# hukenovs/blackman_harris_win

Measured on AMD Instinct MI355X. Metric: window Gsamples/s (BH-7, N=2^26, 32-bit) + fraction of HBM-write roofline, higher is better.
Workload: dtype int64

## Files before the change

blackman_harris_win_amd/csrc/bhw_build.hip:

```cpp
#include "bhw_device.h"

namespace {

template <typename T>
__global__ __launch_bounds__(kBlock) void k_table_build(BhwCordicCfg cfg, uint32_t entries, void *__restrict__ table)
{
    __shared__ T lut_s[32];
    stage_lut<T>(cfg, lut_s);
    const uint32_t u = blockIdx.x * kBlock + threadIdx.x;
    if (u >= entries) return;
    T x, y;
    cordic_q1<T>(lut_s, (T)cfg.x0, (T)((T)u << cfg.z_shl), (int)cfg.n_iter, x, y);
    const int32_t c = (int32_t)(x >> cfg.out_shr), sn = (int32_t)(y >> cfg.out_shr);
    const int2 head = make_int2(__builtin_amdgcn_readfirstlane(c), __builtin_amdgcn_readfirstlane(sn));
    const int4 rec = cfg.tab_dlog > kPackLog ? reinterpret_cast<const int4 *>(cfg.tab_coarse)[u >> fmt_cell_log(cfg.tab_dlog)] : make_int4(0, 0, 0, 0);
    tab_store(table, u, cfg.phi_width - 2 - cfg.z_shr, cfg.tab_split, cfg.tab_dlog, const_cast<void *>(cfg.tab_coarse), c, sn, head, rec,
              cfg.tab_check);
}


template <int NITER, int FMT>
__global__ __launch_bounds__(kBuildThreads) void k_table_build_shared(BhwBuildPlan plan, void *__restrict__ table)
{
    __shared__ int64_t gx[kGroupsPerWg];
    __shared__ int64_t gy[kGroupsPerWg];
    __shared__ int32_t gz[kGroupsPerWg];
    __shared__ int32_t gk[kGroupsPerWg];
    __shared__ uint32_t lut_s[32];
    if (threadIdx.x < 32) lut_s[threadIdx.x] = plan.lut[threadIdx.x];
    __syncthreads();

    constexpr int n_iter = NITER;
    const uint32_t s = plan.z_shl;
    const uint32_t gpw = plan.groups_per_wg;
    const uint32_t group0 = blockIdx.x * gpw;
    const uint32_t n_groups = plan.entries >> 6;

    if (threadIdx.x < gpw) {
        const uint32_t g = group0 + threadIdx.x;
        const uint32_t u_first = g << 6;
        int64_t x = plan.x0, y = plan.x0;
        int32_t zf = (int32_t)((u_first << s) - lut_s[0]);
        const uint32_t span = 63u << s;
        int k = 1;
        bool live = g < n_groups;
        constexpr int kmax = n_iter < kPrefixMax ? n_iter : kPrefixMax;
#pragma unroll
        for (int kk = 1; kk < kmax; ++kk) {
            if (live) {
                const int32_t zl = (int32_t)((uint32_t)zf + span);
                if ((zf < 0) != (zl < 0)) {
                    live = false;
                } else {
                    rot_step(x, y, zf, kk, plan.lut[kk]);
                    k = kk + 1;
                }
            }
        }
        gx[threadIdx.x] = x;
        gy[threadIdx.x] = y;
        gz[threadIdx.x] = zf;
        gk[threadIdx.x] = k;
    }
    __syncthreads();

    const uint32_t wave = __builtin_amdgcn_readfirstlane(threadIdx.x >> 6), lane = threadIdx.x & 63u;
    uint32_t idx_a = lane, idx_m = 64u;
    if (plan.tab_split) {
        const uint32_t e = 1u << plan.log2_entries;
        if (lane & 1u)      { idx_a = (e >> 1) + (lane >> 1); idx_m = 32u; }
        else if (lane & 2u) { idx_a = (e >> 2) + (lane >> 2); idx_m = 16u; }
        else                { idx_a = lane >> 2;              idx_m = 16u; }
    }
    for (uint32_t gi = wave; gi < gpw; gi += kBuildThreads / 64) {
        const uint32_t g = __builtin_amdgcn_readfirstlane(group0 + gi);
        if (g >= n_groups) break;
        int64_t x = gx[gi], y = gy[gi];
        int32_t z = (int32_t)((uint32_t)gz[gi] + (lane << s));
        const int k0 = __builtin_amdgcn_readfirstlane(gk[gi]);
#pragma unroll
        for (int k = 1; k < NITER; ++k) {
            if (k >= kPrefixMax || k >= k0) rot_step(x, y, z, k, plan.lut[k]);
        }
        const int32_t c = (int32_t)(x >> plan.out_shr), sn = (int32_t)(y >> plan.out_shr);
        const int2 head = make_int2(__builtin_amdgcn_readfirstlane(c), __builtin_amdgcn_readfirstlane(sn));
        const uint32_t idx = idx_a + g * idx_m;
        if constexpr (FMT == 4) {
            const uint32_t u = (g << 6) + lane, nmask = 4u * plan.entries - 1u;
            int32_t *d_sin = reinterpret_cast<int32_t *>(table), *d_cos = reinterpret_cast<int32_t *>(const_cast<void *>(plan.tab_coarse));
#pragma unroll
            for (uint32_t q = 0; q < 4u; ++q) {
                int32_t oc, os;
                quadrant_map(q, c, sn, plan.pad0, oc, os);
                const uint32_t i = (q * plan.entries + u - plan.pad) & nmask;
                if (d_sin) d_sin[i] = os;
                if (d_cos) d_cos[i] = oc;
            }
        } else if constexpr (FMT == 0) {
            reinterpret_cast<int2 *>(table)[idx] = make_int2(c, sn);
        } else {
            static_assert(FMT == 1, "k_table_build_shared builds plain and delta16 tables (and the sin / cos sweep) only");
            const int32_t dc = c - head.x, ds = sn - head.y;
            if (plan.check_flag && !(fits_bits(dc, 16) && fits_bits(ds, 16))) atomicOr(plan.check_flag, 1u);
            reinterpret_cast<uint32_t *>(table)[idx] = ((uint32_t)dc & 0xFFFFu) | ((uint32_t)ds << 16);
            if (lane == 0u) reinterpret_cast<int2 *>(const_cast<void *>(plan.tab_coarse))[g] = head;
        }
    }
}

constexpr int kMirrorTail = 6;
constexpr int mirror_gpw(int threads) { return threads / 4; }
constexpr int mirror_heads_max(int threads) { return mirror_gpw(threads) / 2 + 8; }
constexpr int mirror_heads_pad(int threads) { return (mirror_heads_max(threads) + 63) / 64 * 64; }
constexpr int kTailZ = 256;

constexpr int kTailRows = 65;
struct TailD { int8_t v[kTailRows * 64 + 16]; };
constexpr TailD make_tail_d()
{
    TailD t{};
    for (int p = 0; p < 64; ++p)
        for (int v = 0; v < kTailRows; ++v) {
            int d = 0;
            for (int j = 0; j < kMirrorTail; ++j) d += ((p >> j) & 1) ? -(v >> j) : (v >> j);
            t.v[v * 64 + p] = (int8_t)d;
        }
    return t;
}
__device__ const TailD kTailD = make_tail_d();

template <int K, bool ZERO>
__device__ __forceinline__ void rot_narrow(uint32_t &x, uint32_t &y, int32_t &z, uint32_t &zacc, uint32_t lutk)
{
    uint32_t a, b;
    if constexpr (ZERO) {
        asm volatile("v_lshrrev_b32 %[a], %[k], %[y]\n\t"
                     "v_lshrrev_b32 %[b], %[k], %[x]\n\t"
                     "v_min_u32 %[za], %[za], %[z]\n\t"
                     "v_cmpx_gt_i32 vcc, 0, %[z]\n\t"
                     "v_add_u32 %[x], %[x], %[a]\n\t"
                     "v_sub_u32 %[y], %[y], %[b]\n\t"
                     "v_add_u32 %[z], %[z], %[l]\n\t"
                     "s_not_b64 exec, exec\n\t"
                     "v_sub_u32 %[x], %[x], %[a]\n\t"
                     "v_add_u32 %[y], %[y], %[b]\n\t"
                     "v_sub_u32 %[z], %[z], %[l]\n\t"
                     "s_mov_b64 exec, -1"
                     : [x] "+v"(x), [y] "+v"(y), [z] "+v"(z), [za] "+v"(zacc), [a] "=&v"(a), [b] "=&v"(b)
                     : [l] "s"(lutk), [k] "n"(K)
                     : "vcc", "scc");
    } else {
        asm volatile("v_lshrrev_b32 %[a], %[k], %[y]\n\t"
                     "v_lshrrev_b32 %[b], %[k], %[x]\n\t"
                     "v_cmpx_gt_i32 vcc, 0, %[z]\n\t"
                     "v_add_u32 %[x], %[x], %[a]\n\t"
                     "v_sub_u32 %[y], %[y], %[b]\n\t"
                     "v_add_u32 %[z], %[z], %[l]\n\t"
                     "s_not_b64 exec, exec\n\t"
                     "v_sub_u32 %[x], %[x], %[a]\n\t"
                     "v_add_u32 %[y], %[y], %[b]\n\t"
                     "v_sub_u32 %[z], %[z], %[l]\n\t"
                     "s_mov_b64 exec, -1"
                     : [x] "+v"(x), [y] "+v"(y), [z] "+v"(z), [a] "=&v"(a), [b] "=&v"(b)
                     : [l] "s"(lutk), [k] "n"(K)
                     : "vcc", "scc");
    }
}

template <int KA, int NITER>
__device__ __forceinline__ void rot_narrow_block(uint32_t &x, uint32_t &y, int32_t &z, uint32_t &zacc, const uint32_t (&l)[10], int e, uint32_t hi)
{
    uint32_t a, b;
#define BHW_ROT_I(lbl, i, HI_ADD)                                                                                       \
    #lbl ":\n\t"                                                                                                        \
    "v_lshrrev_b32 %[a], %[k" #i "], %[y]\n\t"                                                                          \
    "v_lshrrev_b32 %[b], %[k" #i "], %[x]\n\t"                                                                          \
    HI_ADD                                                                                                             \
    "v_min_u32 %[za], %[za], %[z]\n\t"                                                                                  \
    "v_cmpx_gt_i32 vcc, 0, %[z]\n\t"                                                                                    \
    "v_add_u32 %[x], %[x], %[a]\n\t"                                                                                    \
    "v_sub_u32 %[y], %[y], %[b]\n\t"                                                                                    \
    "v_add_u32 %[z], %[z], %[l" #i "]\n\t"                                                                              \
    "s_not_b64 exec, exec\n\t"                                                                                          \
    "v_sub_u32 %[x], %[x], %[a]\n\t"                                                                                    \
    "v_add_u32 %[y], %[y], %[b]\n\t"                                                                                    \
    "v_sub_u32 %[z], %[z], %[l" #i "]\n\t"                                                                              \
    "s_mov_b64 exec, -1\n"
#define BHW_ROT_PLAIN(i) BHW_ROT_I(i, i, "")
#define BHW_ROT_HI(i) BHW_ROT_I(2##i, i, "v_add_u32 %[b], %[c" #i "], %[b]\n\t")
#define BHW_ROT_DISPATCH(P)                                                                                            \
                 "s_cmp_lt_i32 %[e], 1\n\ts_cbranch_scc1 " #P "0f\n\t"                                                 \
                 "s_cmp_eq_u32 %[e], 1\n\ts_cbranch_scc1 " #P "1f\n\t"                                                 \
                 "s_cmp_eq_u32 %[e], 2\n\ts_cbranch_scc1 " #P "2f\n\t"                                                 \
                 "s_cmp_eq_u32 %[e], 3\n\ts_cbranch_scc1 " #P "3f\n\t"                                                 \
                 "s_cmp_eq_u32 %[e], 4\n\ts_cbranch_scc1 " #P "4f\n\t"                                                 \
                 "s_cmp_eq_u32 %[e], 5\n\ts_cbranch_scc1 " #P "5f\n\t"                                                 \
                 "s_cmp_eq_u32 %[e], 6\n\ts_cbranch_scc1 " #P "6f\n\t"                                                 \
                 "s_cmp_eq_u32 %[e], 7\n\ts_cbranch_scc1 " #P "7f\n\t"                                                 \
                 "s_cmp_eq_u32 %[e], 8\n\ts_cbranch_scc1 " #P "8f\n\t"                                                 \
                 "s_cmp_eq_u32 %[e], 9\n\ts_cbranch_scc1 " #P "9f\n\t"
    constexpr int S = NITER - 1 - KA;
    static_assert(S >= 9 && S <= 30, "bias shifts");
    asm volatile("s_cmp_lg_u32 %[hi], 0\n\ts_cbranch_scc1 100f\n\t"
                 BHW_ROT_DISPATCH()
                 "s_branch 10f\n"
                 BHW_ROT_PLAIN(0) BHW_ROT_PLAIN(1) BHW_ROT_PLAIN(2) BHW_ROT_PLAIN(3) BHW_ROT_PLAIN(4) BHW_ROT_PLAIN(5) BHW_ROT_PLAIN(6) BHW_ROT_PLAIN(7)
                 BHW_ROT_PLAIN(8) BHW_ROT_PLAIN(9)
                 "10:\n\ts_branch 200f\n"
                 "100:\n\t"
                 BHW_ROT_DISPATCH(2)
                 "s_branch 200f\n"
                 BHW_ROT_HI(0) BHW_ROT_HI(1) BHW_ROT_HI(2) BHW_ROT_HI(3) BHW_ROT_HI(4) BHW_ROT_HI(5) BHW_ROT_HI(6) BHW_ROT_HI(7) BHW_ROT_HI(8) BHW_ROT_HI(9)
                 "200:"
                 : [x] "+v"(x), [y] "+v"(y), [z] "+v"(z), [za] "+v"(zacc), [a] "=&v"(a), [b] "=&v"(b)
                 : [e] "s"(e), [hi] "s"(hi), [l0] "s"(l[0]), [l1] "s"(l[1]), [l2] "s"(l[2]), [l3] "s"(l[3]), [l4] "s"(l[4]),
                   [l5] "s"(l[5]), [l6] "s"(l[6]), [l7] "s"(l[7]), [l8] "s"(l[8]), [l9] "s"(l[9]),
                   [k0] "n"(KA), [k1] "n"(KA + 1), [k2] "n"(KA + 2), [k3] "n"(KA + 3), [k4] "n"(KA + 4), [k5] "n"(KA + 5), [k6] "n"(KA + 6),
                   [k7] "n"(KA + 7), [k8] "n"(KA + 8), [k9] "n"(KA + 9),
                   [c0] "n"(1 << S), [c1] "n"(1 << (S - 1)), [c2] "n"(1 << (S - 2)), [c3] "n"(1 << (S - 3)), [c4] "n"(1 << (S - 4)),
                   [c5] "n"(1 << (S - 5)), [c6] "n"(1 << (S - 6)), [c7] "n"(1 << (S - 7)), [c8] "n"(1 << (S - 8)), [c9] "n"(1 << (S - 9))
                 : "vcc", "scc");
#undef BHW_ROT_I
#undef BHW_ROT_PLAIN
#undef BHW_ROT_HI
#undef BHW_ROT_DISPATCH
}

#ifdef BHW_BUILD_STAMPS
__device__ unsigned long long *g_build_stamps = nullptr;
#define BHW_STAMP(i) do { if (g_build_stamps && (threadIdx.x & 63u) == 0u) atomicMax(&g_build_stamps[blockIdx.x * 16u + (i)], (unsigned long long)wall_clock64()); } while (0)
#define BHW_STAMP_MIN(i) do { if (g_build_stamps && threadIdx.x == 0u) g_build_stamps[blockIdx.x * 16u + (i)] = (unsigned long long)wall_clock64(); } while (0)
#else
#define BHW_STAMP(i) do { } while (0)
#define BHW_STAMP_MIN(i) do { } while (0)
#endif

template <int BYTES>
__device__ __forceinline__ void table_store(void *__restrict__ table, uint32_t idx, uint32_t v)
{
    if constexpr (BYTES == 1) asm volatile("global_store_byte %0, %1, %2 sc1" :: "v"(idx), "v"(v), "s"(table) : "memory");
    else asm volatile("global_store_short %0, %1, %2 sc1" :: "v"(idx << 1), "v"(v), "s"(table) : "memory");
}

template <int NITER, int FMT, int THREADS>
__global__ __launch_bounds__(THREADS) __attribute__((amdgpu_waves_per_eu(8, 8))) void k_table_build_mirror(BhwBuildPlan plan, void *__restrict__ table)
{
    BHW_STAMP_MIN(0);
#ifdef BHW_BUILD_STAMPS
    if (g_build_stamps && threadIdx.x == 0u) {
        uint32_t hw, xcc;
        asm volatile("s_getreg_b32 %0, hwreg(HW_REG_HW_ID)\n\ts_getreg_b32 %1, hwreg(HW_REG_XCC_ID)" : "=s"(hw), "=s"(xcc));
        g_build_stamps[blockIdx.x * 16u + 6u] = hw;
        g_build_stamps[blockIdx.x * 16u + 7u] = xcc;
    }
#endif
    static_assert(FMT == 2 || FMT == 3 || FMT == 5, "residual / nibble entries");
    static_assert(NITER >= 21 && NITER <= 32, "narrow state: 32-bit words");
    static_assert(THREADS == 256 || THREADS == 1024, "workgroup shapes");
    constexpr uint32_t gpw = mirror_gpw(THREADS);
    constexpr uint32_t kHeads = mirror_heads_max(THREADS), kHeadsPad = mirror_heads_pad(THREADS);
    static_assert(gpw + 2 * kHeadsPad + 64 <= THREADS, "prefix lanes, two ranges of head chains, the tail-table wave");
    __shared__ int4 gst[gpw];
    __shared__ int2 ghi[gpw];
    __shared__ uint32_t lut_s[32];
    __shared__ uint8_t tail_p[2 * kTailZ];
    __shared__ __attribute__((aligned(16))) int8_t tail_d[kTailRows * 64 + 16];
    constexpr uint32_t kWorkMax = 8 * gpw;
    __shared__ uint32_t work_n;
    __shared__ uint32_t work_u[kWorkMax];
    __shared__ uint32_t esc_n;
    __shared__ int4 esc_list[FMT == 5 ? kEscFill : 1];
    __shared__ int4 esc_tab[FMT == 5 ? kEscSlots : 1];
    if (threadIdx.x < 32) lut_s[threadIdx.x] = plan.lut[threadIdx.x];
    if constexpr (FMT == 5) {
        if (threadIdx.x >= 64u && threadIdx.x < 64u + kEscSlots) esc_tab[threadIdx.x - 64u] = make_int4(-1, 0, 0, 0);
    }
#ifdef BHW_BUILD_STAMPS
    if (g_build_stamps && threadIdx.x == 0u) { asm volatile("s_waitcnt lgkmcnt(0)" ::: "memory"); g_build_stamps[blockIdx.x * 16u + 8u] = (unsigned long long)wall_clock64() | (plan.entries & 0u); }
#endif
    constexpr int n_iter = NITER;
    constexpr int KS = NITER - kMirrorTail;
    const uint32_t s = plan.z_shl;
    const uint32_t group0 = blockIdx.x * gpw;
    const uint32_t E = plan.entries;
    const uint32_t n_groups = E >> 7;
    const uint32_t u_lo = group0 << 6;
    const uint32_t u_hi = ((group0 + gpw) << 6) < (n_groups << 6) ? ((group0 + gpw) << 6) : (n_groups << 6);
    const uint32_t m_last = (E >> 1) - 1u;
    if (threadIdx.x == 0) {
        work_n = 0u;
        esc_n = 0u;
        if (u_hi == (E >> 1)) {
            work_u[0] = E >> 1;
            work_n = 1u;
        }
    }
    if (threadIdx.x >= (uint32_t)THREADS - 64u) {
        const uint32_t t3 = threadIdx.x - ((uint32_t)THREADS - 64u);
#pragma unroll
        for (int q = 0; q < 5; ++q)
            if (t3 + 64u * q < (uint32_t)(kTailRows * 64 + 16) / 16u) reinterpret_cast<int4 *>(tail_d)[t3 + 64u * q] = reinterpret_cast<const int4 *>(kTailD.v)[t3 + 64u * q];
#pragma unroll
        for (int q = 0; q < 2 * kTailZ / 64; ++q) {
            const uint32_t zi = t3 + 64u * (uint32_t)q;
            int32_t z = (int32_t)zi - kTailZ;
            uint32_t p = 0u;
#pragma unroll
            for (int j = 0; j < kMirrorTail; ++j) {
                if (z < 0) { p |= 1u << j; z += (int32_t)plan.lut[KS + j]; } else z -= (int32_t)plan.lut[KS + j];
            }
            tail_p[zi] = (uint8_t)p;
        }
        BHW_STAMP(9);
    }


    __shared__ int32_t hc[2][kHeads], hs[2][kHeads];
    const uint32_t d = fmt_cell_log(plan.tab_dlog);
    const uint32_t cells_total = E >> d;
    uint32_t cell_lo[2] = {0u, 0u}, n_cell[2] = {0u, 0u}, r_lo[2] = {u_lo, 0u}, r_hi[2] = {u_hi, 0u};
    {
        const uint32_t a = u_lo > 1u ? u_lo : 1u, b = (u_hi - 1u) < m_last ? (u_hi - 1u) : m_last;
        if (a <= b) { r_lo[1] = E - b; r_hi[1] = E - a + 1u; }
        if (a <= b && b == (E >> 1) - 1u) r_lo[1] = E >> 1;
    }
#pragma unroll
    for (int w = 0; w < 2; ++w)
        if (r_hi[w] > r_lo[w]) {
            cell_lo[w] = r_lo[w] >> d;
            n_cell[w] = ((r_hi[w] - 1u) >> d) - cell_lo[w] + 1u;
        }
    if (threadIdx.x >= gpw && threadIdx.x < gpw + 2u * kHeadsPad) {
        const uint32_t w = (threadIdx.x - gpw) / kHeadsPad;
        const uint32_t t = (threadIdx.x - gpw) % kHeadsPad;
        if (n_cell[w] && t < n_cell[w] + 2u) {
            const int64_t cell = (t <= n_cell[w]) ? (int64_t)cell_lo[w] + t : (int64_t)cell_lo[w] - 1;
            if (cell >= 0 && cell < (int64_t)cells_total) {
                int64_t x = plan.x0, y = plan.x0;
                int32_t z = (int32_t)((((uint32_t)cell << d) << s) - plan.lut[0]);
#pragma unroll
                for (int r = 1; r < n_iter; ++r) rot_step(x, y, z, r, plan.lut[r]);
                hc[w][t] = (int32_t)(x >> plan.out_shr);
                hs[w][t] = (int32_t)(y >> plan.out_shr);
            }
        }
        BHW_STAMP(10);
    }

    constexpr int kcap = KS < kPrefixMax ? KS : kPrefixMax;
    if (threadIdx.x < gpw) {
        const uint32_t g = group0 + threadIdx.x;
        const uint32_t u_first = g << 6;
        int64_t x = plan.x0, y = plan.x0;
        int32_t zf = (int32_t)((u_first << s) - plan.lut[0]);
        const uint32_t span = 63u << s;
        int k = 1;
        bool live = g < n_groups;
        uint32_t zero0 = 0u;
#pragma unroll
        for (int kk = 1; kk < kcap; ++kk) {
            if (live) {
                const int32_t zl = (int32_t)((uint32_t)zf + span);
                if ((zf < 0) != (zl < 0)) {
                    live = false;
                } else {
                    zero0 |= (uint32_t)(zf == 0);
                    rot_step(x, y, zf, kk, plan.lut[kk]);
                    k = kk + 1;
                }
            }
        }
        const int64_t drift = ((int64_t)1 << (NITER - k + 1)) + 2, lim = (int64_t)1 << NITER;
        const bool narrow = x >= drift && y >= drift && x + drift < lim && y + drift < lim;
        constexpr int64_t kBias = (int64_t)1 << (NITER - 1);
        const bool hi = !narrow && k >= KS - 10 && y >= drift && y + drift < lim && x - kBias >= drift && x - kBias + drift < ((int64_t)1 << 32) &&
                        x + drift < lim + ((int64_t)1 << KS);
        const int64_t xp = hi ? x - kBias : x;
        const uint32_t flags = zero0 | (narrow || hi ? 2u : 0u) | (hi ? 4u : 0u) | (g == 0u ? 8u : 0u);
        gst[threadIdx.x] = make_int4((int32_t)xp, (int32_t)y, zf, (int32_t)((uint32_t)k | (flags << 8)));
        ghi[threadIdx.x] = make_int2((int32_t)(xp >> 32), (int32_t)(y >> 32));
        BHW_STAMP(11);
    }
    BHW_STAMP(1);
    __syncthreads();

    __shared__ int4 hrec[2][kHeads];
    {
        const uint32_t w = threadIdx.x / kHeadsPad, t = threadIdx.x % kHeadsPad;
        if (w < 2u && t < n_cell[w]) {
            const uint32_t cell = cell_lo[w] + t;
            int4 r;
            if (cell + 1u < cells_total) r = make_int4(hc[w][t], hs[w][t], hc[w][t + 1] - hc[w][t], hs[w][t + 1] - hs[w][t]);
            else {
                const uint32_t tp = t ? t - 1u : n_cell[w] + 1u;
                r = make_int4(hc[w][t], hs[w][t], hc[w][t] - hc[w][tp], hs[w][t] - hs[w][tp]);
            }
            if constexpr (FMT == 5) { r.x += (int32_t)kEscBias; r.y += (int32_t)kEscBias; }
            if constexpr (fmt_is_nibble(FMT)) { r.x -= 8; r.y -= 8; }
            hrec[w][t] = r;
            if constexpr (fmt_is_nibble(FMT)) { r.z *= 2; r.w *= 2; }
            if ((cell << d) >= r_lo[w])
                reinterpret_cast<int4 *>(const_cast<void *>(plan.tab_coarse))[cell] = r;
        }
    }
    __syncthreads();
    BHW_STAMP_MIN(2);
    auto record_of = [&](int w, uint32_t cell) -> int4 { return hrec[w][cell - cell_lo[w]]; };

    auto store_entry = [&](auto CHECKED, uint32_t idx, int32_t c, int32_t sn, const int4 rec, uint32_t pos) {
        if constexpr (FMT == 5) {
            const int2 p = tab_predict(rec, pos, d);
            const uint32_t nc = (uint32_t)(c - p.x), ns = (uint32_t)(sn - p.y);
            uint32_t v = nc | (ns << 4);
            if (__builtin_expect((int)(nc - 1u > 14u) | (int)(ns > 15u), 0)) {
                const uint32_t slot = atomicAdd(&esc_n, 1u);
                if (slot < kEscFill) esc_list[slot] = make_int4((int32_t)idx, c, sn, 0);
                v = kEscMarker;
            }
            table_store<1>(table, idx, v);
        } else if constexpr (FMT == 3) {
            const int2 p = tab_predict(rec, pos, d);
            const uint32_t nc = (uint32_t)(c - p.x), ns = (uint32_t)(sn - p.y);
            if constexpr (decltype(CHECKED)::value) {
                if (plan.check_flag && (nc | ns) > 15u) atomicOr(plan.check_flag, 1u);
            }
            table_store<1>(table, idx, nc | (ns << 4));
        } else {
            const int2 p = tab_predict(rec, pos, d);
            const int32_t dc = c - p.x, ds = sn - p.y;
            if constexpr (decltype(CHECKED)::value) {
                if (plan.check_flag && !(fits_bits(dc, 8) && fits_bits(ds, 8))) atomicOr(plan.check_flag, 1u);
            }
            table_store<2>(table, idx, ((uint32_t)dc & 0xFFu) | ((uint32_t)ds << 8));
        }
    };

    const uint32_t wave = __builtin_amdgcn_readfirstlane(threadIdx.x >> 6), lane = threadIdx.x & 63u;
    uint32_t idx_a, idx_m, idx_i;
    if (lane & 1u)      { idx_a = (E >> 1) + (lane >> 1); idx_m = 32u; idx_i = E + (E >> 1) - 1u; }
    else if (lane & 2u) { idx_a = (E >> 2) + (lane >> 2); idx_m = 16u; idx_i = (E >> 1) + (E >> 2) - 1u; }
    else                { idx_a = lane >> 2;              idx_m = 16u; idx_i = E >> 2; }
    if (!plan.tab_split) { idx_a = lane; idx_m = 64u; idx_i = E; }
    const uint32_t fmask = (1u << d) - 1u;
    constexpr uint32_t kWaves = THREADS / 64;
    static_assert(gpw == 16u * kWaves, "a wave walks 16 groups: four at each priority");
    constexpr bool kWholeCells = THREADS % (1 << 9) == 0;
    const uint32_t gi_end = group0 >= n_groups ? 0u : n_groups - group0 < gpw ? n_groups - group0 : gpw;
    const uint32_t zlane = lane << s;
    const uint32_t cell_step = ((uint32_t)THREADS >> d) << 4;
    constexpr int KA = KS - 10;
    static_assert(KA >= 5 && KA < kcap && KS - KA == 10, "ten-rotation block");
    uint32_t rom[10];
#pragma unroll
    for (int i = 0; i < 10; ++i) {
        rom[i] = __builtin_amdgcn_readfirstlane(lut_s[KA + i]);
        asm volatile("" : "+s"(rom[i]));
    }
    auto build_groups = [&](auto CHECKED) {
        uint32_t u = ((group0 + wave) << 6) + lane;
        uint32_t st_off = wave * (uint32_t)sizeof(int4);
        asm volatile("" : "+v"(st_off));
        uint32_t idx = idx_a + (group0 + wave) * idx_m;
        uint32_t off1, pos1, off2, pos2;
        auto cells_of = [&]() {
            const uint32_t um = E - u;
            pos1 = u & fmask;
            off1 = ((u >> d) - cell_lo[0]) << 4;
            pos2 = um & fmask;
            off2 = ((um >> d) - cell_lo[1]) << 4;
        };
        cells_of();
        uint32_t gi = wave;
#pragma unroll 1
        for (uint32_t quarter = 0; quarter < 4u; ++quarter) {
            if (quarter == 0u) __builtin_amdgcn_s_setprio(3);
            else if (quarter == 1u) __builtin_amdgcn_s_setprio(2);
            else if (quarter == 2u) __builtin_amdgcn_s_setprio(1);
            else __builtin_amdgcn_s_setprio(0);
            const uint32_t q_end = (quarter + 1u) * 4u * kWaves < gi_end ? (quarter + 1u) * 4u * kWaves : gi_end;
#pragma unroll 1
            for (; gi < q_end; gi += kWaves) {
                const int4 st = *reinterpret_cast<const int4 *>(reinterpret_cast<const char *>(gst) + st_off);
                const uint32_t kf = __builtin_amdgcn_readfirstlane((uint32_t)st.w);
                const int k0 = (int)(kf & 0xFFu);
                const uint32_t gf = kf >> 8;
                int32_t z = (int32_t)((uint32_t)st.z + zlane);
                uint64_t zmask = 0ull;
                int32_t c1, s1, c2, s2;
                if (gf & 2u) {
                    uint32_t x = (uint32_t)st.x, y = (uint32_t)st.y;
                    uint32_t zacc = ~0u;
                    if (k0 < KA) {
#define BHW_NARROW(K) if constexpr (K < KA) { if (K >= k0) rot_narrow<K, true>(x, y, z, zacc, K < 9 ? (uint32_t)__builtin_amdgcn_readfirstlane(lut_s[K]) : plan.lut[K]); }
                        BHW_NARROW(1) BHW_NARROW(2) BHW_NARROW(3) BHW_NARROW(4) BHW_NARROW(5) BHW_NARROW(6) BHW_NARROW(7) BHW_NARROW(8)
                        BHW_NARROW(9) BHW_NARROW(10) BHW_NARROW(11) BHW_NARROW(12) BHW_NARROW(13) BHW_NARROW(14) BHW_NARROW(15)
#undef BHW_NARROW
                    }
                    const uint32_t hi = (gf >> 2) & 1u;
                    rot_narrow_block<KA, NITER>(x, y, z, zacc, rom, k0 - KA, hi);
                    zmask = __builtin_amdgcn_ballot_w64(zacc == 0u);
                    const uint32_t xrow6 = hi << (NITER - 1 - KS + 6);
                    const uint32_t bias_out = (hi << (NITER - 1)) >> plan.out_shr;
                    static_assert(KS <= 26, "unrolled to rotation 25");
                    constexpr uint32_t lowm = (1u << KS) - 1u;
                    const uint32_t zi = (uint32_t)(z + kTailZ);
                    const uint32_t mx = (x + 128u) & lowm, my = (y + 128u) & lowm;
                    const uint32_t unsafe = (uint32_t)((mx < my ? mx : my) < 256u) | (uint32_t)((zi - 1u) >= (uint32_t)(2 * kTailZ - 1));
                    if (__builtin_expect(__builtin_amdgcn_ballot_w64(unsafe != 0u) == 0ull, 1)) {
                        const uint32_t xx = ((x >> KS) << 6) + xrow6, yy = (y >> KS) << 6;
                        const uint32_t p1 = tail_p[zi], p2 = tail_p[2u * kTailZ - zi];
                        const int32_t dx1 = tail_d[p1 + yy], dy1 = tail_d[p1 + xx], dx2 = tail_d[p2 + xx], dy2 = tail_d[p2 + yy];
                        c1 = (int32_t)(((x - (uint32_t)dx1) >> plan.out_shr) + bias_out);
                        s1 = (int32_t)((y + (uint32_t)dy1) >> plan.out_shr);
                        c2 = (int32_t)((y - (uint32_t)dx2) >> plan.out_shr);
                        s2 = (int32_t)(((x + (uint32_t)dy2) >> plan.out_shr) + bias_out);
                    } else if (hi) {
                        int64_t xw = (int64_t)x + ((int64_t)1 << (NITER - 1)), yw = (int64_t)y;
                        int64_t x2 = yw, y2 = xw;
                        int32_t z2 = -z;
#pragma unroll 1
                        for (int k = KS; k < NITER; ++k) {
                            rot_step_dyn(xw, yw, z, k, lut_s[k], true);
                            rot_step_dyn(x2, y2, z2, k, lut_s[k], true);
                        }
                        c1 = (int32_t)(xw >> plan.out_shr); s1 = (int32_t)(yw >> plan.out_shr);
                        c2 = (int32_t)(x2 >> plan.out_shr); s2 = (int32_t)(y2 >> plan.out_shr);
                    } else {
                        uint32_t x2 = y, y2 = x;
                        int32_t z2 = -z;
                        uint32_t unused = 0u;
#define BHW_NARROW(K) if constexpr (K >= KS && K < NITER) { rot_narrow<K, false>(x, y, z, unused, plan.lut[K]); rot_narrow<K, false>(x2, y2, z2, unused, plan.lut[K]); }
                        BHW_NARROW(15) BHW_NARROW(16) BHW_NARROW(17) BHW_NARROW(18) BHW_NARROW(19) BHW_NARROW(20) BHW_NARROW(21) BHW_NARROW(22)
                        BHW_NARROW(23) BHW_NARROW(24) BHW_NARROW(25) BHW_NARROW(26) BHW_NARROW(27) BHW_NARROW(28) BHW_NARROW(29) BHW_NARROW(30)
                        BHW_NARROW(31)
#undef BHW_NARROW
                        c1 = (int32_t)(x >> plan.out_shr); s1 = (int32_t)(y >> plan.out_shr);
                        c2 = (int32_t)(x2 >> plan.out_shr); s2 = (int32_t)(y2 >> plan.out_shr);
                    }
                } else {
                    const int2 high = ghi[gi];
                    int64_t x = (int64_t)(((uint64_t)(uint32_t)high.x << 32) | (uint32_t)st.x), y = (int64_t)(((uint64_t)(uint32_t)high.y << 32) | (uint32_t)st.y);
#pragma unroll 1
                    for (int k = k0; k < KS; ++k) {
                        zmask |= __builtin_amdgcn_ballot_w64(z == 0);
                        rot_step_dyn(x, y, z, k, lut_s[k], k >= kMad24From);
                    }
                    int64_t x2 = y, y2 = x;
                    int32_t z2 = -z;
#pragma unroll 1
                    for (int k = KS; k < NITER; ++k) {
                        rot_step_dyn(x, y, z, k, lut_s[k], true);
                        rot_step_dyn(x2, y2, z2, k, lut_s[k], true);
                    }
                    c1 = (int32_t)(x >> plan.out_shr); s1 = (int32_t)(y >> plan.out_shr);
                    c2 = (int32_t)(x2 >> plan.out_shr); s2 = (int32_t)(y2 >> plan.out_shr);
                }
                const uint32_t own_idx = fmt_is_nibble(FMT) ? u : idx;
                store_entry(CHECKED, own_idx, c1, s1, *reinterpret_cast<const int4 *>(reinterpret_cast<const char *>(hrec[0]) + off1), pos1);
                auto store_image = [&]() {
                    store_entry(CHECKED, fmt_is_nibble(FMT) ? E - u : idx_i - idx, c2, s2,
                                *reinterpret_cast<const int4 *>(reinterpret_cast<const char *>(hrec[1]) + off2), pos2);
                };
                const uint32_t events = (uint32_t)zmask | (uint32_t)(zmask >> 32) | (gf & 9u);
                if (events == 0u) {
                    store_image();
                } else {
                    const bool replay = u != 0u && ((((zmask >> lane) & 1ull) != 0ull) || ((gf & 1u) && lane == 0u));
                    bool deferred = false;
                    if (replay) {
                        const uint32_t slot = atomicAdd(&work_n, 1u);
                        if (slot < kWorkMax) { work_u[slot] = u; deferred = true; }
                        else {
                            int64_t xf = plan.x0, yf = plan.x0;
                            int32_t zf = (int32_t)(((E - u) << s) - lut_s[0]);
#pragma unroll 1
                            for (int r = 1; r < n_iter; ++r) rot_step_dyn(xf, yf, zf, r, lut_s[r], r >= kMad24From);
                            c2 = (int32_t)(xf >> plan.out_shr);
                            s2 = (int32_t)(yf >> plan.out_shr);
                        }
                    }
                    if (u != 0u && !deferred) store_image();
                }
                u += (uint32_t)THREADS;
                st_off += kWaves * (uint32_t)sizeof(int4);
                idx += kWaves * idx_m;
                if constexpr (kWholeCells) { off1 += cell_step; off2 -= cell_step; }
                else cells_of();
            }
        }
    };
    if constexpr (FMT == 5) build_groups(std::false_type{});
    else if (plan.check_flag) build_groups(std::true_type{});
    else build_groups(std::false_type{});
    BHW_STAMP_MIN(3);
    BHW_STAMP(4);
    __syncthreads();
    const uint32_t n_work = work_n < kWorkMax ? work_n : kWorkMax;
    for (uint32_t i = threadIdx.x; i < n_work; i += THREADS) {
        const uint32_t um = E - work_u[i];
        int64_t xf = plan.x0, yf = plan.x0;
        int32_t zf = (int32_t)((um << s) - plan.lut[0]);
#pragma unroll
        for (int r = 1; r < n_iter; ++r) rot_step(xf, yf, zf, r, plan.lut[r]);
        store_entry(std::true_type{}, tab_index(um, plan.log2_entries, plan.tab_split), (int32_t)(xf >> plan.out_shr), (int32_t)(yf >> plan.out_shr), record_of(1, um >> d), um & fmask);
    }
    if constexpr (FMT == 5) {
        __syncthreads();
        const uint32_t n_esc = esc_n < kEscFill ? esc_n : kEscFill;
        uint32_t tid = threadIdx.x;
        asm volatile("" : "+v"(tid));
        if (tid < n_esc) {
            const int4 it = esc_list[tid];
            uint32_t h = esc_slot((uint32_t)it.x);
#pragma unroll 1
            for (uint32_t i = 0; i < kEscSlots; ++i) {
                const uint32_t was = atomicCAS(reinterpret_cast<uint32_t *>(&esc_tab[h].x), ~0u, (uint32_t)it.x);
                if (was == ~0u || was == (uint32_t)it.x) { esc_tab[h].y = it.y; esc_tab[h].z = it.z; break; }
                h = (h + 1u) & (kEscSlots - 1u);
            }
        }
        __syncthreads();
        if (tid < kEscSlots) reinterpret_cast<int4 *>(plan.tab_esc)[(size_t)blockIdx.x * kEscSlots + tid] = esc_tab[tid];
        if (tid == 0u && esc_n > kEscFill && plan.check_flag) atomicOr(plan.check_flag, 1u);
    }
    BHW_STAMP(5);
}

template <int NITER>
__global__ __launch_bounds__(kBlock) void k_table_build_plain(BhwCordicCfg cfg, uint32_t entries, int2 *__restrict__ table)
{
    __shared__ uint32_t lut_s[32];
    if (threadIdx.x < 32) lut_s[threadIdx.x] = (uint32_t)cfg.lut[threadIdx.x];
    __syncthreads();
    const uint32_t u = blockIdx.x * kBlock + threadIdx.x;
    if (u >= entries) return;
    int64_t x = cfg.x0, y = cfg.x0;
    int32_t z = (int32_t)((u << cfg.z_shl) - lut_s[0]);
#pragma unroll
    for (int r = 1; r < NITER; ++r) rot_step(x, y, z, r, lut_s[r]);
    table[u] = make_int2((int32_t)(x >> cfg.out_shr), (int32_t)(y >> cfg.out_shr));
}

}


int bhwk_sincos_sweep(const BhwLaunch &l, const BhwCordicCfg &c, uint64_t theta0, int32_t *d_sin, int32_t *d_cos)
{
    hipStream_t st = (hipStream_t)l.stream;
    BhwBuildPlan plan;
    for (uint32_t k = 0; k < 32; ++k) plan.lut[k] = (uint32_t)c.lut[k];
    plan.entries = 1u << (c.phi_width - 2);
    plan.n_iter = c.n_iter;
    plan.z_shl = c.z_shl;
    plan.out_shr = c.out_shr;
    plan.log2_entries = c.phi_width - 2;
    plan.tab_split = 0;
    plan.tab_dlog = 0;
    plan.pad0 = c.ones_neg;
    plan.tab_coarse = d_cos;
    plan.x0 = c.x0;
    plan.check_flag = nullptr;
    plan.tab_esc = nullptr;
    const unsigned groups = plan.entries >> 6;
    plan.groups_per_wg = groups >= 64u * 1024u ? 64u : groups >= 16u * 1024u ? 16u : 4u;
    plan.pad = (uint32_t)(theta0 & ((1ull << c.phi_width) - 1ull));
    const dim3 grid((groups + plan.groups_per_wg - 1) / plan.groups_per_wg), block(kBuildThreads);
    if (!with_int_range<7, 32>(c.n_iter, [&](auto N) { launch(k_table_build_shared<N, 4>, grid, block, st, plan, (void *)d_sin); }))
        return (int)hipErrorInvalidValue;
    return finish(hipSuccess);
}

#ifdef BHW_BUILD_STAMPS
extern "C" int bhw_dbg_build_stamps(void *d_words)
{
    unsigned long long *p = (unsigned long long *)d_words;
    return (int)hipMemcpyToSymbol(HIP_SYMBOL(g_build_stamps), &p, sizeof p);
}
#endif

int bhwk_table_build(const BhwLaunch &l, const BhwCordicCfg &c_in, int32_t *d_table)
{
    const BhwCordicCfg c = table_layout(c_in);
    hipStream_t st = (hipStream_t)l.stream;
    const uint32_t entries = 1u << (c.phi_width - 2 - c.z_shr);
    const bool fits = (c.dat_width + c.out_shr <= 34);
    if (fits && c.n_iter >= 7 && entries < (1u << 20) && c.tab_dlog == 0 && !c.tab_split) {
        const dim3 grid(grid_for(entries)), block(kBlock);
        if (!with_int_range<7, 32>(c.n_iter, [&](auto N) { launch(k_table_build_plain<N>, grid, block, st, c, entries, (int2 *)d_table); }))
            return (int)hipErrorInvalidValue;
        return finish(hipSuccess);
    }
    if (entries >= 64 && fits && c.n_iter >= 2) {
        BhwBuildPlan plan;
        for (uint32_t k = 0; k < 32; ++k) plan.lut[k] = (uint32_t)c.lut[k];
        plan.entries = entries;
        plan.n_iter = c.n_iter;
        plan.z_shl = c.z_shl;
        plan.out_shr = c.out_shr;
        plan.log2_entries = c.phi_width - 2 - c.z_shr;
        plan.tab_split = c.tab_split;
        plan.tab_dlog = c.tab_dlog;
        plan.pad0 = 0;
        plan.tab_coarse = c.tab_coarse;
        plan.x0 = c.x0;
        plan.check_flag = c.tab_check;
        plan.tab_esc = const_cast<void *>(c.tab_esc);
        const unsigned groups = entries >> 6;
        plan.groups_per_wg = groups >= 64u * 1024u ? 64u : groups >= 16u * 1024u ? 16u : 4u;
        plan.pad = 0;
        const dim3 grid((groups + plan.groups_per_wg - 1) / plan.groups_per_wg), block(kBuildThreads);
        const int fmt = fmt_of(c.tab_dlog);
        if (c.n_iter < 21 && fmt != 0) return (int)hipErrorInvalidValue;
        if (bhwk_build_mirror_applies(c, entries)) {
            const unsigned own_groups = entries >> 7;
            const unsigned threads = bhwk_build_mirror_threads(entries);
            const unsigned mgpw = (unsigned)mirror_gpw((int)threads);
            const dim3 mgrid((own_groups + mgpw - 1) / mgpw), mblock(threads);
            plan.groups_per_wg = mgpw;
            const bool listed = with_int_range<21, 32>(c.n_iter, [&](auto N) {
                with_int_or_last<2, 3, 5>(fmt, [&](auto F) {
                    with_int_or_last<1024, 256>((int)threads, [&](auto T) {
                        launch(k_table_build_mirror<N, F, T>, mgrid, mblock, st, plan, (void *)d_table);
                    });
                });
            });
            return listed ? finish(hipSuccess) : (int)hipErrorInvalidValue;
        }
        if (fmt > 1) return (int)hipErrorInvalidValue;
        const bool listed = with_int_range<7, 32>(c.n_iter, [&](auto N) {
            if constexpr (N < 21) launch(k_table_build_shared<N, 0>, grid, block, st, plan, (void *)d_table);
            else with_int_or_last<0, 1>(fmt, [&](auto F) { launch(k_table_build_shared<N, F>, grid, block, st, plan, (void *)d_table); });
        });
        return listed ? finish(hipSuccess) : (int)hipErrorInvalidValue;
    }
    if (c.tab_dlog > kPackLog) return (int)hipErrorInvalidValue;
    if (c.wide) launch(k_table_build<int64_t>, dim3(grid_for(entries)), dim3(kBlock), st, c, entries, (void *)d_table);
    else        launch(k_table_build<int32_t>, dim3(grid_for(entries)), dim3(kBlock), st, c, entries, (void *)d_table);
    return finish(hipSuccess);
}
```

Baseline: 729.3.

## Precompute first four CORDIC rotations per group as ranked candidates

For groups whose 64 lanes share the starting rotation index, the setup phase now enumerates all 16 outcomes of the next four CORDIC micro-rotations and stores them in shared memory. It also stores a 64-bit lane mask of where each threshold crossing falls. In the build loop each lane finds its candidate with mbcnt over that mask, replacing four serialized rotations with one LDS lookup plus z-offset and zero-accumulator corrections. The ten-rotation dispatch is also reordered into a two-level branch to shorten the compare chain. The cost is more shared memory and setup work per group, plus a monotonicity check that falls back to the old path when it fails.

```diff
diff --git a/blackman_harris_win_amd/csrc/bhw_build.hip b/blackman_harris_win_amd/csrc/bhw_build.hip
--- a/blackman_harris_win_amd/csrc/bhw_build.hip
+++ b/blackman_harris_win_amd/csrc/bhw_build.hip
@@ -128,6 +128,30 @@
     return t;
 }
 __device__ const TailD kTailD = make_tail_d();
+
+constexpr int kRankSkip = 4;
+constexpr int kRankCand = (1 << kRankSkip) + 1;
+template <typename L>
+__device__ __forceinline__ int32_t rank_threshold(uint32_t p, const L &l)
+{
+    int32_t t = 0;
+#pragma unroll
+    for (int m = 0; m + 1 < kRankSkip; ++m) {
+        const uint32_t bit = 1u << (kRankSkip - 1 - m);
+        if (p & (bit - 1u)) t += (p & bit) ? (int32_t)l[m] : -(int32_t)l[m];
+    }
+    return t;
+}
+template <int M, int R>
+__device__ __forceinline__ void rank_candidates(uint32_t x, uint32_t y, uint32_t k, uint32_t bk, uint2 *out)
+{
+    if constexpr (M == kRankSkip) out[R] = make_uint2(x, y);
+    else {
+        const uint32_t a = y >> k, b = (x >> k) + bk;
+        rank_candidates<M + 1, 2 * R>(x + a, y - b, k + 1u, bk >> 1, out);
+        rank_candidates<M + 1, 2 * R + 1>(x - a, y + b, k + 1u, bk >> 1, out);
+    }
+}
 
 template <int K, bool ZERO>
 __device__ __forceinline__ void rot_narrow(uint32_t &x, uint32_t &y, int32_t &z, uint32_t &zacc, uint32_t lutk)
@@ -188,12 +212,14 @@
     "s_mov_b64 exec, -1\n"
 #define BHW_ROT_PLAIN(i) BHW_ROT_I(i, i, "")
 #define BHW_ROT_HI(i) BHW_ROT_I(2##i, i, "v_add_u32 %[b], %[c" #i "], %[b]\n\t")
-#define BHW_ROT_DISPATCH(P)                                                                                            \
+#define BHW_ROT_DISPATCH(P, H)                                                                                         \
+                 "s_cmp_gt_i32 %[e], 4\n\ts_cbranch_scc1 " #H "f\n\t"                                                 \
                  "s_cmp_lt_i32 %[e], 1\n\ts_cbranch_scc1 " #P "0f\n\t"                                                 \
                  "s_cmp_eq_u32 %[e], 1\n\ts_cbranch_scc1 " #P "1f\n\t"                                                 \
                  "s_cmp_eq_u32 %[e], 2\n\ts_cbranch_scc1 " #P "2f\n\t"                                                 \
                  "s_cmp_eq_u32 %[e], 3\n\ts_cbranch_scc1 " #P "3f\n\t"                                                 \
-                 "s_cmp_eq_u32 %[e], 4\n\ts_cbranch_scc1 " #P "4f\n\t"                                                 \
+                 "s_branch " #P "4f\n"                                                                                  \
+                 #H ":\n\t"                                                                                            \
                  "s_cmp_eq_u32 %[e], 5\n\ts_cbranch_scc1 " #P "5f\n\t"                                                 \
                  "s_cmp_eq_u32 %[e], 6\n\ts_cbranch_scc1 " #P "6f\n\t"                                                 \
                  "s_cmp_eq_u32 %[e], 7\n\ts_cbranch_scc1 " #P "7f\n\t"                                                 \
@@ -202,13 +228,13 @@
     constexpr int S = NITER - 1 - KA;
     static_assert(S >= 9 && S <= 30, "bias shifts");
     asm volatile("s_cmp_lg_u32 %[hi], 0\n\ts_cbranch_scc1 100f\n\t"
-                 BHW_ROT_DISPATCH()
+                 BHW_ROT_DISPATCH(, 40)
                  "s_branch 10f\n"
                  BHW_ROT_PLAIN(0) BHW_ROT_PLAIN(1) BHW_ROT_PLAIN(2) BHW_ROT_PLAIN(3) BHW_ROT_PLAIN(4) BHW_ROT_PLAIN(5) BHW_ROT_PLAIN(6) BHW_ROT_PLAIN(7)
                  BHW_ROT_PLAIN(8) BHW_ROT_PLAIN(9)
                  "10:\n\ts_branch 200f\n"
                  "100:\n\t"
-                 BHW_ROT_DISPATCH(2)
+                 BHW_ROT_DISPATCH(2, 41)
                  "s_branch 200f\n"
                  BHW_ROT_HI(0) BHW_ROT_HI(1) BHW_ROT_HI(2) BHW_ROT_HI(3) BHW_ROT_HI(4) BHW_ROT_HI(5) BHW_ROT_HI(6) BHW_ROT_HI(7) BHW_ROT_HI(8) BHW_ROT_HI(9)
                  "200:"
@@ -265,6 +291,9 @@
     __shared__ uint32_t lut_s[32];
     __shared__ uint8_t tail_p[2 * kTailZ];
     __shared__ __attribute__((aligned(16))) int8_t tail_d[kTailRows * 64 + 16];
+    constexpr bool kRank = THREADS == 1024 || FMT != 5;
+    __shared__ uint2 cand_s[kRank ? gpw * kRankCand : 1];
+    __shared__ int2 rank_tab[kRank ? 8 << kRankSkip : 1];
     constexpr uint32_t kWorkMax = 8 * gpw;
     __shared__ uint32_t work_n;
     __shared__ uint32_t work_u[kWorkMax];
@@ -280,6 +309,9 @@
 #endif
     constexpr int n_iter = NITER;
     constexpr int KS = NITER - kMirrorTail;
+    constexpr int KA = KS - 10;
+    constexpr int kRankTop = KS - kRankSkip < kPrefixMax ? KS - kRankSkip : kPrefixMax;
+    static_assert(kRankTop - KA < 8 && kRankTop + kRankSkip <= 31, "rank_tab rows; ROM words");
     const uint32_t s = plan.z_shl;
     const uint32_t group0 = blockIdx.x * gpw;
     const uint32_t E = plan.entries;
@@ -311,6 +343,16 @@
             }
             tail_p[zi] = (uint8_t)p;
         }
+        if (kRank && t3 < (1u << kRankSkip)) {
+#pragma unroll
+            for (int row = 0; row <= kRankTop - KA; ++row) {
+                const uint32_t l[kRankSkip] = {plan.lut[KA + row], plan.lut[KA + row + 1], plan.lut[KA + row + 2], plan.lut[KA + row + 3]};
+                int32_t off = 0;
+#pragma unroll
+                for (int m = 0; m < kRankSkip; ++m) off += (t3 >> (kRankSkip - 1 - m)) & 1u ? (int32_t)l[m] : -(int32_t)l[m];
+                rank_tab[(row << kRankSkip) + t3] = make_int2(off, t3 ? rank_threshold(t3, l) : INT32_MIN);
+            }
+        }
         BHW_STAMP(9);
     }
 
@@ -376,8 +418,40 @@
         const bool hi = !narrow && k >= KS - 10 && y >= drift && y + drift < lim && x - kBias >= drift && x - kBias + drift < ((int64_t)1 << 32) &&
                         x + drift < lim + ((int64_t)1 << KS);
         const int64_t xp = hi ? x - kBias : x;
-        const uint32_t flags = zero0 | (narrow || hi ? 2u : 0u) | (hi ? 4u : 0u) | (g == 0u ? 8u : 0u);
-        gst[threadIdx.x] = make_int4((int32_t)xp, (int32_t)y, zf, (int32_t)((uint32_t)k | (flags << 8)));
+        uint32_t flags = zero0 | (narrow || hi ? 2u : 0u) | (hi ? 4u : 0u) | (g == 0u ? 8u : 0u);
+        uint32_t w0 = (uint32_t)xp, w1 = (uint32_t)y, kw = (uint32_t)k;
+        if (kRank && (narrow || hi) && k >= KA && k <= kRankTop) {
+            uint32_t l[kRankSkip - 1] = {};
+#pragma unroll
+            for (int kk = KA; kk <= kRankTop; ++kk)
+                if (k == kk) {
+#pragma unroll
+                    for (int m = 0; m + 1 < kRankSkip; ++m) l[m] = plan.lut[kk + m];
+                }
+            uint64_t mask = 0ull;
+            uint32_t below = 0u, above = 0u;
+            bool ok = true;
+            int32_t prev = INT32_MIN;
+            const int32_t round_up = (int32_t)((1u << s) - 1u) - zf;
+#pragma unroll
+            for (uint32_t p = 1; p < (1u << kRankSkip); ++p) {
+                const int32_t t = rank_threshold(p, l);
+                ok = ok && t > prev;
+                prev = t;
+                const int32_t first = (t + round_up) >> s;
+                if (first <= 0) ++below;
+                else if (first > 63) ++above;
+                else mask |= 1ull << (first - 1);
+            }
+            if (ok && (uint32_t)__builtin_popcountll(mask) + below + above == (1u << kRankSkip) - 1u) {
+                rank_candidates<0, 0>((uint32_t)xp, (uint32_t)y, (uint32_t)k, hi ? 1u << (NITER - 1 - k) : 0u, &cand_s[threadIdx.x * kRankCand]);
+                w0 = (uint32_t)mask;
+                w1 = (uint32_t)(mask >> 32);
+                kw = (uint32_t)(k + kRankSkip) | (below << 16) | ((uint32_t)(k - KA) << (20 + kRankSkip + 3));
+                flags |= 16u;
+            }
+        }
+        gst[threadIdx.x] = make_int4((int32_t)w0, (int32_t)w1, zf, (int32_t)(kw | (flags << 8)));
         ghi[threadIdx.x] = make_int2((int32_t)(xp >> 32), (int32_t)(y >> 32));
         BHW_STAMP(11);
     }
@@ -448,7 +522,6 @@
     const uint32_t gi_end = group0 >= n_groups ? 0u : n_groups - group0 < gpw ? n_groups - group0 : gpw;
     const uint32_t zlane = lane << s;
     const uint32_t cell_step = ((uint32_t)THREADS >> d) << 4;
-    constexpr int KA = KS - 10;
     static_assert(KA >= 5 && KA < kcap && KS - KA == 10, "ten-rotation block");
     uint32_t rom[10];
 #pragma unroll
@@ -460,6 +533,8 @@
         uint32_t u = ((group0 + wave) << 6) + lane;
         uint32_t st_off = wave * (uint32_t)sizeof(int4);
         asm volatile("" : "+v"(st_off));
+        uint32_t cand_off = wave * (uint32_t)(kRankCand * sizeof(uint2));
+        asm volatile("" : "+v"(cand_off));
         uint32_t idx = idx_a + (group0 + wave) * idx_m;
         uint32_t off1, pos1, off2, pos2;
         auto cells_of = [&]() {
@@ -483,14 +558,22 @@
                 const int4 st = *reinterpret_cast<const int4 *>(reinterpret_cast<const char *>(gst) + st_off);
                 const uint32_t kf = __builtin_amdgcn_readfirstlane((uint32_t)st.w);
                 const int k0 = (int)(kf & 0xFFu);
-                const uint32_t gf = kf >> 8;
+                const uint32_t gf = (kf >> 8) & 0xFFu;
                 int32_t z = (int32_t)((uint32_t)st.z + zlane);
                 uint64_t zmask = 0ull;
                 int32_t c1, s1, c2, s2;
                 if (gf & 2u) {
                     uint32_t x = (uint32_t)st.x, y = (uint32_t)st.y;
                     uint32_t zacc = ~0u;
-                    if (k0 < KA) {
+                    if (kRank && (gf & 16u)) {
+                        const uint32_t rank = __builtin_amdgcn_mbcnt_hi((uint32_t)st.y, __builtin_amdgcn_mbcnt_lo((uint32_t)st.x, ((uint32_t)st.w >> 16) & 15u));
+                        const uint2 cs = *reinterpret_cast<const uint2 *>(reinterpret_cast<const char *>(cand_s) + cand_off + (rank << 3));
+                        const int2 rt = *reinterpret_cast<const int2 *>(reinterpret_cast<const char *>(rank_tab) + ((uint32_t)st.w >> 20) + (rank << 3));
+                        zacc = (uint32_t)z - (uint32_t)rt.y;
+                        z -= rt.x;
+                        x = cs.x;
+                        y = cs.y;
+                    } else if (k0 < KA) {
 #define BHW_NARROW(K) if constexpr (K < KA) { if (K >= k0) rot_narrow<K, true>(x, y, z, zacc, K < 9 ? (uint32_t)__builtin_amdgcn_readfirstlane(lut_s[K]) : plan.lut[K]); }
                         BHW_NARROW(1) BHW_NARROW(2) BHW_NARROW(3) BHW_NARROW(4) BHW_NARROW(5) BHW_NARROW(6) BHW_NARROW(7) BHW_NARROW(8)
                         BHW_NARROW(9) BHW_NARROW(10) BHW_NARROW(11) BHW_NARROW(12) BHW_NARROW(13) BHW_NARROW(14) BHW_NARROW(15)
@@ -583,6 +666,7 @@
                 }
                 u += (uint32_t)THREADS;
                 st_off += kWaves * (uint32_t)sizeof(int4);
+                cand_off += kWaves * (uint32_t)(kRankCand * sizeof(uint2));
                 idx += kWaves * idx_m;
                 if constexpr (kWholeCells) { off1 += cell_step; off2 -= cell_step; }
                 else cells_of();
```

Result: faster. 756.2 (median of 6 runs) (+3.7%).
